# HandSomeWay/myGauHuman

Hardware: AMD Instinct MI355X
Metric: frames/sec fwd+bwd @1024^2, 200k Gaussians (higher is better)
Workload: dtype f32

## Files before the change

### mygauhuman_amd/csrc/geometry.hip

```cpp
#include "expand.h"
#include "gsr_common.h"
#include "project.h"
#include "sh_math.h"

namespace gsr {

constexpr int SH_M = 16;
constexpr int SH_ROW = SH_M * 3;
constexpr int SH_HALF = SH_ROW / 2;
constexpr int SH_LDS_ROW = 28;
constexpr int SH_CPT = SH_HALF / 4;

template <bool STAGE_SH>
__global__ __launch_bounds__(PRE_BLOCK) void preprocess_forward_kernel(const PreprocessArgs a) {
  __shared__ uint32_t wave_tot[PRE_BLOCK / WAVE];
  __shared__ __attribute__((aligned(16))) float s_sh[STAGE_SH ? PRE_BLOCK * SH_LDS_ROW : 4];
  const int i = blockIdx.x * PRE_BLOCK + threadIdx.x;
  float4 second[STAGE_SH ? SH_CPT : 1];
  if (STAGE_SH) {
    const int first = blockIdx.x * PRE_BLOCK;
    const int nrows = min(PRE_BLOCK, a.P - first);
    if (a.sh_half) {
      const uint4 *slab = reinterpret_cast<const uint4 *>(reinterpret_cast<const _Float16 *>(a.shs) + (size_t)first * SH_ROW);
#pragma unroll
// ... 54 lines not shown
        const float l1 = mid + sqrtf(fmaxf(0.1f, mid * mid - det));
        const float l2 = mid - sqrtf(fmaxf(0.1f, mid * mid - det));
        const float radf = ceilf(3.f * sqrtf(fmaxf(l1, l2)));
        const float pix = ndc2pix(pprojx, a.W), piy = ndc2pix(pprojy, a.H);
        int x0, y0, x1, y1;
        const int radi = f2i_sat(radf);
        tile_rect(pix, piy, radi, a.grid_x, a.grid_y, x0, y0, x1, y1);
        const uint32_t area = (uint32_t)(x1 - x0) * (uint32_t)(y1 - y0);
        if (area != 0) {
          float3 rgb = make_float3(0.f, 0.f, 0.f);
          if (a.colors_precomp) {
            rgb = make_float3(a.colors_precomp[3 * (size_t)i], a.colors_precomp[3 * (size_t)i + 1], a.colors_precomp[3 * (size_t)i + 2]);
          } else if (STAGE_SH) {
            want_sh = true;
          } else {
            rgb = sh_to_rgb(a.D, p, a.campos, a.shs + (size_t)i * a.M * 3, clamp_bits);
          }
          my_radius = radi;
          tiles = area;
          rec.x = pix;
          rec.y = piy;
          rec.conic_a = cv.z * det_inv;
          rec.conic_b = -cv.y * det_inv;
          rec.conic_c = cv.x * det_inv;
          rec.opacity = a.opacities[i];
          rec.depth = pv.z;
          rec.r = rgb.x;
          rec.g = rgb.y;
          rec.b = rgb.z;
          const float o = rec.opacity, t255 = 255.0f * o;
          float hx = __builtin_inff(), hy = __builtin_inff();
// ... 4 lines not shown
              const float tau2 = 2.0f * (logf(t255) + 0.02f);
              hx = sqrtf(tau2 * cv.x) * 1.0001f + 0.01f;
              hy = sqrtf(tau2 * cv.z) * 1.0001f + 0.01f;
            }
          }
          rec.hx = hx;
          rec.hy = hy;
        }
      }
    }
  }
  if (STAGE_SH) {
    float3 d0;
    const ShDir dir = sh_dir(p, a.campos, d0);
    float res[3] = {0.f, 0.f, 0.f};
    __syncthreads();
    if (want_sh) sh_accumulate<0, SH_M / 2>(a.D, dir, &s_sh[threadIdx.x * SH_LDS_ROW], res);
    __syncthreads();
    {
      const int nrows = min(PRE_BLOCK, a.P - blockIdx.x * PRE_BLOCK);
      if (a.sh_half) {
#pragma unroll
        for (int j = 0; j < SH_CPT / 2; j++) {
          const int e = (int)threadIdx.x + j * PRE_BLOCK, row = e / (SH_CPT / 2), c8 = e % (SH_CPT / 2);
          if (row < nrows) {
            const _Float16 *hv = reinterpret_cast<const _Float16 *>(&second[j]);
            float *dst = &s_sh[row * SH_LDS_ROW + 8 * c8];
#pragma unroll
            for (int e2 = 0; e2 < 8; e2++) dst[e2] = (float)hv[e2];
          }
        }
      } else {
#pragma unroll
        for (int j = 0; j < SH_CPT; j++) {
          const int e = (int)threadIdx.x + j * PRE_BLOCK, row = e / SH_CPT, c4 = e % SH_CPT;
          if (row < nrows) *reinterpret_cast<float4 *>(&s_sh[row * SH_LDS_ROW + 4 * c4]) = second[j];
        }
      }
    }
    __syncthreads();
    if (want_sh) {
      sh_accumulate<SH_M / 2, SH_M>(a.D, dir, &s_sh[threadIdx.x * SH_LDS_ROW], res);
      const float3 rgb = sh_finish(res, clamp_bits);
      rec.r = rgb.x;
      rec.g = rgb.y;
      rec.b = rgb.z;
    }
  }
  if (i < a.P) {
    a.radii[i] = my_radius;
    a.geom.tiles_touched[i] = tiles;
    a.geom.clamped[i] = (uint8_t)clamp_bits;
    float4 *dst = reinterpret_cast<float4 *>(a.geom.recs + i);
    dst[0] = make_float4(rec.x, rec.y, rec.conic_a, rec.conic_b);
    dst[1] = make_float4(rec.conic_c, rec.opacity, rec.depth, rec.r);
    dst[2] = make_float4(rec.g, rec.b, rec.hx, rec.hy);
    if (a.zero_rows) {
      float4 *row = reinterpret_cast<float4 *>(a.geom.grad_rows + (size_t)i * GROWX);
#pragma unroll
      for (int k = 0; k < GROWX / 4; k++) row[k] = make_float4(0.f, 0.f, 0.f, 0.f);
    }
// ... 137 lines not shown
```

### mygauhuman_amd/csrc/gsr_api.hip

```cpp
#include <stdarg.h>
#include <stdio.h>
#include <string.h>

#include <atomic>
#include <mutex>
#include <string>
#include <unordered_map>
#include <utility>
#include <vector>

#include "gsr_common.h"

namespace gsr {

static thread_local std::string g_error;

void set_error(const char *fmt, ...) {
  char buf[1024];
  va_list ap;
  va_start(ap, fmt);
  vsnprintf(buf, sizeof(buf), fmt, ap);
  va_end(ap);
  g_error = buf;
}
// ... 638 lines not shown
      !dL_dcov3D) {
    set_error("gsr_rasterize_backward: null required pointer");
    return GSR_EINVAL;
  }
  if (p1 && (n_extra != CE_MAX || !p1->gt_image || !p1->gt_normal || !p1->alpha_target || !p1->bound || !p1->color || !p1->alpha ||
             !p1->extra_images || !p1->stats || p1->normal_triple < 0 || p1->normal_triple > 5 || p1->axis_triple < 0 ||
             p1->axis_triple > 5 || p1->axis_triple == p1->normal_triple)) {
    set_error("gsr_rasterize_backward_phase1_loss: the fused multi-feature pass (n_extra = %d), the forward's images, the targets, "
              "the bound mask, stats and two different triple indices in 0..5 are required", CE_MAX);
    return GSR_EINVAL;
  }
  if ((shs && !dL_dsh) || (scales && (!rotations || !dL_dscale || !dL_drot))) {
    set_error("gsr_rasterize_backward: missing gradient output for SH / scale / rotation inputs");
    return GSR_EINVAL;
  }
  const int grid_x = (width + TILE - 1) / TILE, grid_y = (height + TILE - 1) / TILE;
  const size_t tiles = (size_t)grid_x * grid_y, npix = (size_t)width * height;
  GeomState geom = geom_from_chunk(geom_buffer, (size_t)P);
  BinningState bin = binning_from_chunk(binning_buffer, (size_t)R);
  ImageState img = image_from_chunk(image_buffer, npix, tiles);
  if (!radii) radii = geom.internal_radii;

  if (n_extra != 0 && (n_extra != CE_MAX || !extra_features || !dL_dout_extra || !dL_dextra)) {
    set_error("gsr_rasterize_backward_ex: extra feature channels need n_extra == %d and all three arrays", CE_MAX);
    return GSR_EINVAL;
  }
  const int grow = n_extra ? GROWX : GROW;
  const Options opt = options_for(stream);
  float *det_rows = nullptr;
  const size_t det_bytes = (size_t)(R > 0 ? R : 1) * 4 * GROW * sizeof(float);
// ... 68 lines not shown
      (void)hipFree(det_rows);
    }
    return rc;
  }
  GSR_LAUNCH_CHECK(stream, debug);

  PreprocessBwdArgs pb;
  memset(&pb, 0, sizeof(pb));
  pb.P = P;
  pb.D = D;
  pb.M = M;
  pb.means3D = means3D;
  pb.shs = shs;
  pb.scales = scales;
  pb.rotations = rotations;
  pb.cov3D = cov3D_precomp ? cov3D_precomp : geom.cov3D;
  pb.radii = radii;
  pb.clamped = geom.clamped;
  pb.scale_modifier = scale_modifier;
  pb.view = viewmatrix;
  pb.proj = projmatrix;
  pb.campos = campos;
  pb.W = width;
  pb.H = height;
  pb.tan_fovx = tan_fovx;
  pb.tan_fovy = tan_fovy;
  pb.focal_y = height / (2.0f * tan_fovy);
  pb.focal_x = width / (2.0f * tan_fovx);
  pb.grad_rows = geom.grad_rows;
  pb.grow = grow;
  pb.clear_rows = (flags & GSR_BWD_ROWS_ZEROED) ? 1 : 0;
  pb.CE = n_extra;
  pb.sh_half = sh_dtype == GSR_SH_F16 ? 1 : 0;
// ... 257 lines not shown
```

### mygauhuman_amd/csrc/gsr_common.h

```cpp
#pragma once
#include <hip/hip_runtime.h>
#include <stdint.h>
#include <stddef.h>

#include "../../include/gsr.h"

namespace gsr {

constexpr int TILE = 16;
constexpr int WAVE = 64;
constexpr int PRE_BLOCK = 256;

struct alignas(16) SplatRec {
  float x, y, conic_a, conic_b;
  float conic_c, opacity, depth, r;
  float g, b, hx, hy;
};
static_assert(sizeof(SplatRec) == 48, "SplatRec layout");

constexpr int GROW = 16;

constexpr int GROWX = 32;
constexpr int CE_MAX = 18;

struct GeomState {
  SplatRec *recs;
  float *cov3D;
  uint8_t *clamped;
  uint32_t *tiles_touched;
  uint32_t *point_offsets;
  int *internal_radii;
  uint32_t *block_incl;
  uint32_t *block_sums;
  uint32_t *block_prefix;
  uint32_t *total;
  float *grad_rows;
};
struct BinningState {
  uint64_t *keys_a;
  uint32_t *vals_a;
  uint64_t *keys_s;
  uint32_t *vals_s;
  uint32_t *hist;
// ... 20 lines not shown

inline int pre_blocks(int P) { return (P + PRE_BLOCK - 1) / PRE_BLOCK; }
constexpr int SORT_ITEMS = 16;
constexpr int SORT_BLOCK = 256;
constexpr int SORT_TILE = SORT_ITEMS * SORT_BLOCK;
inline size_t sort_blocks(size_t n) { return (n + SORT_TILE - 1) / SORT_TILE; }
inline size_t sort_hist_words(size_t n) { return 256 * (sort_blocks(n) ? sort_blocks(n) : 1) + 256; }

inline GeomState geom_from_chunk(char *chunk_, size_t P, size_t *end = nullptr) {
  GeomState g;
  uintptr_t chunk = carve_begin(chunk_);
  size_t nb = (size_t)pre_blocks((int)P);
  carve(chunk, g.recs, P);
  carve(chunk, g.cov3D, P * 6);
  carve(chunk, g.clamped, P);
  carve(chunk, g.tiles_touched, P);
  carve(chunk, g.point_offsets, P);
  carve(chunk, g.internal_radii, P);
  carve(chunk, g.block_incl, P);
  carve(chunk, g.block_sums, nb);
  carve(chunk, g.block_prefix, nb);
  carve(chunk, g.total, 4);
  carve(chunk, g.grad_rows, P * GROWX);
  if (end) *end = chunk;
  return g;
}
inline size_t geom_bytes(size_t P) {
  size_t end = 0;
  geom_from_chunk(nullptr, P, &end);
  return end + 256;
// ... 225 lines not shown
  const float *g_img[CB_IMAGES];
  int n_img;
  uint64_t col0;
  uint32_t col_mask;
  float *dL_dextra;
  float *dL_dcolor;
  int list_prio;
};
int launch_blend_colors_backward(const BlendColorsBwdArgs &a, hipStream_t stream);

struct PreprocessBwdArgs {
  int P, D, M;
  const float *means3D, *shs, *scales, *rotations, *cov3D;
  const int *radii;
  const uint8_t *clamped;
  float scale_modifier;
  const float *view, *proj, *campos;
  int W, H;
  float tan_fovx, tan_fovy, focal_x, focal_y;
  float *grad_rows;
  int grow;
  int clear_rows;
  int CE;
  float *dL_dextra;
  const SplatRec *recs;
  float *dL_dmean2D, *dL_dconic, *dL_dopacity, *dL_dcolor, *dL_dmean3D, *dL_dcov3D, *dL_dsh, *dL_dscale, *dL_drot;
  int sh_half;
};
int launch_preprocess_backward(const PreprocessBwdArgs &a, hipStream_t stream);

// ... 104 lines not shown
```

### mygauhuman_amd/csrc/preprocess_bwd.hip

```cpp
#include "gsr_common.h"
#include "sh_math.h"

namespace gsr {

__device__ __forceinline__ void cov3d_backward(const float3 sc, float mod, const float4 q, const float *d, float *dL_dscale,
                                               float *dL_drot) {
  const float r = q.x, x = q.y, y = q.z, z = q.w;
  float R[3][3];
  R[0][0] = 1.f - 2.f * (y * y + z * z);
  R[0][1] = 2.f * (x * y - r * z);
  R[0][2] = 2.f * (x * z + r * y);
  R[1][0] = 2.f * (x * y + r * z);
  R[1][1] = 1.f - 2.f * (x * x + z * z);
  R[1][2] = 2.f * (y * z - r * x);
  R[2][0] = 2.f * (x * z - r * y);
  R[2][1] = 2.f * (y * z + r * x);
  R[2][2] = 1.f - 2.f * (x * x + y * y);
  const float s[3] = {mod * sc.x, mod * sc.y, mod * sc.z};
  float M[3][3];
#pragma unroll
  for (int c = 0; c < 3; c++)
#pragma unroll
    for (int rr = 0; rr < 3; rr++) M[c][rr] = s[rr] * R[c][rr];
  const float dS[3][3] = {{d[0], 0.5f * d[1], 0.5f * d[2]}, {0.5f * d[1], d[3], 0.5f * d[4]}, {0.5f * d[2], 0.5f * d[4], d[5]}};
// ... 6 lines not shown
#pragma unroll
  for (int k = 0; k < 3; k++) dL_dscale[k] = R[0][k] * dMt[k][0] + R[1][k] * dMt[k][1] + R[2][k] * dMt[k][2];
#pragma unroll
  for (int k = 0; k < 3; k++)
#pragma unroll
    for (int rr = 0; rr < 3; rr++) dMt[k][rr] *= s[k];
  dL_drot[0] = 2 * z * (dMt[0][1] - dMt[1][0]) + 2 * y * (dMt[2][0] - dMt[0][2]) + 2 * x * (dMt[1][2] - dMt[2][1]);
  dL_drot[1] = 2 * y * (dMt[1][0] + dMt[0][1]) + 2 * z * (dMt[2][0] + dMt[0][2]) + 2 * r * (dMt[1][2] - dMt[2][1]) -
               4 * x * (dMt[2][2] + dMt[1][1]);
  dL_drot[2] = 2 * x * (dMt[1][0] + dMt[0][1]) + 2 * r * (dMt[2][0] - dMt[0][2]) + 2 * z * (dMt[1][2] + dMt[2][1]) -
               4 * y * (dMt[2][2] + dMt[0][0]);
  dL_drot[3] = 2 * r * (dMt[0][1] - dMt[1][0]) + 2 * x * (dMt[2][0] + dMt[0][2]) + 2 * y * (dMt[1][2] + dMt[2][1]) -
               4 * z * (dMt[1][1] + dMt[0][0]);
}

struct DeferredSh {
  bool live;
  float3 mean;
  float dRGB[3];
  float dm[3];
};

template <bool DEFER_SH>
__device__ __forceinline__ void preprocess_backward_one(const PreprocessBwdArgs &a, int i, const float *sh_in, float *dsh_out,
                                                        DeferredSh *out) {
  if (DEFER_SH) out->live = false;
  if (!(a.radii[i] > 0)) {
#pragma unroll
    for (int k = 0; k < 3; k++) {
      a.dL_dmean2D[3 * (size_t)i + k] = 0.f;
      a.dL_dcolor[3 * (size_t)i + k] = 0.f;
      a.dL_dmean3D[3 * (size_t)i + k] = 0.f;
      if (a.scales) a.dL_dscale[3 * (size_t)i + k] = 0.f;
    }
#pragma unroll
    for (int k = 0; k < 4; k++) {
      a.dL_dconic[4 * (size_t)i + k] = 0.f;
      if (a.scales) a.dL_drot[4 * (size_t)i + k] = 0.f;
    }
    a.dL_dopacity[i] = 0.f;
// ... 28 lines not shown
  a.dL_dmean2D[3 * (size_t)i + 1] = g0.y;
  a.dL_dmean2D[3 * (size_t)i + 2] = 0.f;
  a.dL_dconic[4 * (size_t)i + 0] = g0.z;
  a.dL_dconic[4 * (size_t)i + 1] = g0.w;
  a.dL_dconic[4 * (size_t)i + 2] = 0.f;
  a.dL_dconic[4 * (size_t)i + 3] = g1.x;
  a.dL_dopacity[i] = g1.y;
  a.dL_dcolor[3 * (size_t)i + 0] = g1.z;
  a.dL_dcolor[3 * (size_t)i + 1] = g1.w;
  a.dL_dcolor[3 * (size_t)i + 2] = g2.x;
  const float dcx = g0.z, dcy = g0.w, dcz = g1.x;

  const float *vm = a.view, *proj = a.proj;
  const float3 mean = make_float3(a.means3D[3 * (size_t)i], a.means3D[3 * (size_t)i + 1], a.means3D[3 * (size_t)i + 2]);
  float c6[6];
#pragma unroll
  for (int k = 0; k < 6; k++) c6[k] = a.cov3D[6 * (size_t)i + k];

  float3 t = make_float3(vm[0] * mean.x + vm[4] * mean.y + vm[8] * mean.z + vm[12],
                         vm[1] * mean.x + vm[5] * mean.y + vm[9] * mean.z + vm[13],
                         vm[2] * mean.x + vm[6] * mean.y + vm[10] * mean.z + vm[14]);
  const float limx = 1.3f * a.tan_fovx, limy = 1.3f * a.tan_fovy;
  const float txtz = t.x / t.z, tytz = t.y / t.z;
  t.x = fminf(limx, fmaxf(-limx, txtz)) * t.z;
  t.y = fminf(limy, fmaxf(-limy, tytz)) * t.z;
  const float gxm = (txtz < -limx || txtz > limx) ? 0.f : 1.f;
  const float gym = (tytz < -limy || tytz > limy) ? 0.f : 1.f;
  const float h_x = a.focal_x, h_y = a.focal_y;
  const float J00 = h_x / t.z, J02 = -(h_x * t.x) / (t.z * t.z), J11 = h_y / t.z, J12 = -(h_y * t.y) / (t.z * t.z);
  const float Wm[3][3] = {{vm[0], vm[4], vm[8]}, {vm[1], vm[5], vm[9]}, {vm[2], vm[6], vm[10]}};
  float T[2][3];
#pragma unroll
// ... 49 lines not shown
  const float dtz = -h_x * tz2 * dJ00 - h_y * tz2 * dJ11 + (2 * h_x * t.x) * tz3 * dJ02 + (2 * h_y * t.y) * tz3 * dJ12;
  float dm[3];
  dm[0] = vm[0] * dtx + vm[1] * dty + vm[2] * dtz;
  dm[1] = vm[4] * dtx + vm[5] * dty + vm[6] * dtz;
  dm[2] = vm[8] * dtx + vm[9] * dty + vm[10] * dtz;

  const float mhw = proj[3] * mean.x + proj[7] * mean.y + proj[11] * mean.z + proj[15];
  const float m_w = 1.0f / (mhw + 0.0000001f);
  const float mul1 = (proj[0] * mean.x + proj[4] * mean.y + proj[8] * mean.z + proj[12]) * m_w * m_w;
  const float mul2 = (proj[1] * mean.x + proj[5] * mean.y + proj[9] * mean.z + proj[13]) * m_w * m_w;
  const float g2x = g0.x, g2y = g0.y;
  dm[0] += (proj[0] * m_w - proj[3] * mul1) * g2x + (proj[1] * m_w - proj[3] * mul2) * g2y;
  dm[1] += (proj[4] * m_w - proj[7] * mul1) * g2x + (proj[5] * m_w - proj[7] * mul2) * g2y;
  dm[2] += (proj[8] * m_w - proj[11] * mul1) * g2x + (proj[9] * m_w - proj[11] * mul2) * g2y;

  if (DEFER_SH) {
    const uint32_t cb = a.clamped[i];
    out->live = true;
    out->mean = mean;
    out->dRGB[0] = (cb & 1u) ? 0.f : g1.z;
    out->dRGB[1] = (cb & 2u) ? 0.f : g1.w;
    out->dRGB[2] = (cb & 4u) ? 0.f : g2.x;
    out->dm[0] = dm[0];
    out->dm[1] = dm[1];
    out->dm[2] = dm[2];
  } else {
    if (a.shs) {
      sh_backward(a.D, mean, a.campos, sh_in, a.clamped[i], make_float3(g1.z, g1.w, g2.x), dm, dsh_out);
      for (int k = (a.D + 1) * (a.D + 1) * 3; k < a.M * 3; k++) dsh_out[k] = 0.f;
    }
    a.dL_dmean3D[3 * (size_t)i + 0] = dm[0];
    a.dL_dmean3D[3 * (size_t)i + 1] = dm[1];
    a.dL_dmean3D[3 * (size_t)i + 2] = dm[2];
  }

  if (a.scales) {
    float ds[3], dq[4];
    const float3 sc = make_float3(a.scales[3 * (size_t)i], a.scales[3 * (size_t)i + 1], a.scales[3 * (size_t)i + 2]);
    const float4 q = make_float4(a.rotations[4 * (size_t)i], a.rotations[4 * (size_t)i + 1], a.rotations[4 * (size_t)i + 2],
                                 a.rotations[4 * (size_t)i + 3]);
    cov3d_backward(sc, a.scale_modifier, q, dcov, ds, dq);
#pragma unroll
    for (int k = 0; k < 3; k++) a.dL_dscale[3 * (size_t)i + k] = ds[k];
#pragma unroll
    for (int k = 0; k < 4; k++) a.dL_drot[4 * (size_t)i + k] = dq[k];
  }
}

constexpr int BSH_M = 16, BSH_ROW = BSH_M * 3;
constexpr int BSH_HALF = BSH_ROW / 2;
constexpr int BSH_LDS_ROW = 28;
constexpr int BSH_CPT = BSH_HALF / 4;
constexpr int BWD_BLOCK = 128;

template <bool STAGE_SH>
__global__ __launch_bounds__(BWD_BLOCK) void preprocess_backward_kernel(const PreprocessBwdArgs a) {
  __shared__ __attribute__((aligned(16))) float s_sh[STAGE_SH ? BWD_BLOCK * BSH_LDS_ROW : 4];
  const int i = blockIdx.x * BWD_BLOCK + threadIdx.x;
  if (a.CE > 0) {
    const int first = blockIdx.x * BWD_BLOCK;
    const int nrows = min(BWD_BLOCK, a.P - first);
    const float *src = a.grad_rows + (size_t)first * a.grow + 9;
    float *dst = a.dL_dextra + (size_t)first * a.CE;
    for (int e = threadIdx.x; e < nrows * a.CE; e += BWD_BLOCK) {
      const int r = e / a.CE, c = e - r * a.CE;
      dst[e] = src[(size_t)r * a.grow + c];
    }
    if (a.clear_rows) {
      __syncthreads();
      float *rows = a.grad_rows + (size_t)first * a.grow;
      for (int e = threadIdx.x; e < nrows * (a.grow - 12); e += BWD_BLOCK) {
        const int r = e / (a.grow - 12), c = e - r * (a.grow - 12);
        rows[(size_t)r * a.grow + 12 + c] = 0.f;
      }
    }
  }
  if (STAGE_SH) {
    const int first = blockIdx.x * BWD_BLOCK;
    const int nrows = min(BWD_BLOCK, a.P - first);
    float4 second[BSH_CPT];
    if (a.sh_half) {
      const uint4 *slab = reinterpret_cast<const uint4 *>(reinterpret_cast<const _Float16 *>(a.shs) + (size_t)first * BSH_ROW);
#pragma unroll
      for (int j = 0; j < BSH_CPT / 2; j++) {
        const int e = (int)threadIdx.x + j * BWD_BLOCK, row = e / (BSH_CPT / 2), c8 = e % (BSH_CPT / 2);
        if (row < nrows) {
          const uint4 v = slab[row * (BSH_ROW / 8) + c8];
          second[j] = __builtin_bit_cast(float4, slab[row * (BSH_ROW / 8) + BSH_CPT / 2 + c8]);
          const _Float16 *hv = reinterpret_cast<const _Float16 *>(&v);
          float *dst = &s_sh[row * BSH_LDS_ROW + 8 * c8];
#pragma unroll
          for (int e2 = 0; e2 < 8; e2++) dst[e2] = (float)hv[e2];
        }
      }
    } else {
      const float4 *slab = reinterpret_cast<const float4 *>(a.shs + (size_t)first * BSH_ROW);
#pragma unroll
      for (int j = 0; j < BSH_CPT; j++) {
        const int e = (int)threadIdx.x + j * BWD_BLOCK, row = e / BSH_CPT, c4 = e % BSH_CPT;
        if (row < nrows) {
          *reinterpret_cast<float4 *>(&s_sh[row * BSH_LDS_ROW + 4 * c4]) = slab[row * (BSH_ROW / 4) + c4];
          second[j] = slab[row * (BSH_ROW / 4) + BSH_CPT + c4];
        }
      }
    }
    DeferredSh d;
    d.live = false;
    if (i < a.P) preprocess_backward_one<true>(a, i, nullptr, nullptr, &d);
    float3 d0 = make_float3(1.f, 0.f, 0.f);
    ShDir dir = {};
    float dd[9] = {0.f, 0.f, 0.f, 0.f, 0.f, 0.f, 0.f, 0.f, 0.f};
    if (d.live) dir = sh_dir(d.mean, a.campos, d0);
    float *mine = &s_sh[threadIdx.x * BSH_LDS_ROW];
    float4 *out = reinterpret_cast<float4 *>(a.dL_dsh + (size_t)first * BSH_ROW);
    __syncthreads();
    if (d.live) {
      sh_backward_range<0, BSH_M / 2>(a.D, dir, mine, d.dRGB, dd);
    } else if (i < a.P) {
#pragma unroll
      for (int k = 0; k < BSH_HALF; k++) mine[k] = 0.f;
    }
    __syncthreads();
#pragma unroll
    for (int j = 0; j < BSH_CPT; j++) {
      const int e = (int)threadIdx.x + j * BWD_BLOCK, row = e / BSH_CPT, c4 = e % BSH_CPT;
      if (row < nrows) {
        float4 *cell = reinterpret_cast<float4 *>(&s_sh[row * BSH_LDS_ROW + 4 * c4]);
        out[row * (BSH_ROW / 4) + c4] = *cell;
        if (!a.sh_half) *cell = second[j];
      }
    }
    if (a.sh_half) {
      __syncthreads();
#pragma unroll
      for (int j = 0; j < BSH_CPT / 2; j++) {
        const int e = (int)threadIdx.x + j * BWD_BLOCK, row = e / (BSH_CPT / 2), c8 = e % (BSH_CPT / 2);
        if (row < nrows) {
          const _Float16 *hv = reinterpret_cast<const _Float16 *>(&second[j]);
          float *dst = &s_sh[row * BSH_LDS_ROW + 8 * c8];
#pragma unroll
          for (int e2 = 0; e2 < 8; e2++) dst[e2] = (float)hv[e2];
        }
      }
    }
    __syncthreads();
    if (d.live) {
      sh_backward_range<BSH_M / 2, BSH_M>(a.D, dir, mine, d.dRGB, dd);
      sh_backward_finish(d0, d.dRGB, dd, d.dm);
      a.dL_dmean3D[3 * (size_t)i + 0] = d.dm[0];
      a.dL_dmean3D[3 * (size_t)i + 1] = d.dm[1];
      a.dL_dmean3D[3 * (size_t)i + 2] = d.dm[2];
    } else if (i < a.P) {
#pragma unroll
      for (int k = 0; k < BSH_HALF; k++) mine[k] = 0.f;
    }
    __syncthreads();
#pragma unroll
    for (int j = 0; j < BSH_CPT; j++) {
      const int e = (int)threadIdx.x + j * BWD_BLOCK, row = e / BSH_CPT, c4 = e % BSH_CPT;
      if (row < nrows) out[row * (BSH_ROW / 4) + BSH_CPT + c4] = *reinterpret_cast<const float4 *>(&s_sh[row * BSH_LDS_ROW + 4 * c4]);
    }
  } else {
    if (i < a.P)
      preprocess_backward_one<false>(a, i, a.shs ? a.shs + (size_t)i * a.M * 3 : nullptr,
                                     a.shs ? a.dL_dsh + (size_t)i * a.M * 3 : nullptr, nullptr);
  }
}

int launch_preprocess_backward(const PreprocessBwdArgs &a, hipStream_t stream) {
  if (a.P <= 0) return GSR_OK;
  const bool stage = a.shs && a.M == BSH_M && (reinterpret_cast<size_t>(a.shs) % 16 == 0) &&
                     (reinterpret_cast<size_t>(a.dL_dsh) % 16 == 0);
  if (a.sh_half && a.shs && !stage) {
    set_error("fp16 SH storage needs 16 coefficients per Gaussian and 16-byte aligned arrays");
    return GSR_EINVAL;
  }
  if (stage)
    hipLaunchKernelGGL(preprocess_backward_kernel<true>, dim3((a.P + BWD_BLOCK - 1) / BWD_BLOCK), dim3(BWD_BLOCK), 0, stream, a);
  else
    hipLaunchKernelGGL(preprocess_backward_kernel<false>, dim3((a.P + BWD_BLOCK - 1) / BWD_BLOCK), dim3(BWD_BLOCK), 0, stream, a);
  return GSR_OK;
}

}
```

### mygauhuman_amd/csrc/sh_math.h

```cpp
#pragma once
#include "gsr_common.h"

namespace gsr {

constexpr float kSH0 = 0.28209479177387814f;
constexpr float kSH1 = 0.4886025119029199f;
constexpr float kSH2[5] = {1.0925484305920792f, -1.0925484305920792f, 0.31539156525252005f, -1.0925484305920792f,
                           0.5462742152960396f};
constexpr float kSH3[7] = {-0.5900435899266435f, 2.890611442640554f, -0.4570457994644658f, 0.3731763325901154f,
                           -0.4570457994644658f, 1.445305721320277f,  -0.5900435899266435f};

__device__ __forceinline__ float3 sh_to_rgb(int deg, const float3 pos, const float *campos, const float *sh,
                                            uint32_t &clamp_bits) {
  const float dx0 = pos.x - campos[0], dy0 = pos.y - campos[1], dz0 = pos.z - campos[2];
  const float len = sqrtf(dx0 * dx0 + dy0 * dy0 + dz0 * dz0);
  const float x = dx0 / len, y = dy0 / len, z = dz0 / len;
  float out[3];
  clamp_bits = 0;
#pragma unroll
  for (int ch = 0; ch < 3; ch++) {
#define S(k) sh[(k) * 3 + ch]
    float res = kSH0 * S(0);
    if (deg > 0) {
      res = res - kSH1 * y * S(1) + kSH1 * z * S(2) - kSH1 * x * S(3);
// ... 175 lines not shown
    sh_accumulate<LO, HI, K + 1>(deg, d, part, res);
  }
}
__device__ __forceinline__ float3 sh_finish(float (&res)[3], uint32_t &clamp_bits) {
  clamp_bits = 0;
#pragma unroll
  for (int ch = 0; ch < 3; ch++) {
    res[ch] += 0.5f;
    if (res[ch] < 0) clamp_bits |= 1u << ch;
    res[ch] = fmaxf(res[ch], 0.0f);
  }
  return make_float3(res[0], res[1], res[2]);
}

template <int LO, int HI, int K = LO>
__device__ __forceinline__ void sh_backward_range(int deg, const ShDir &d, float *part, const float (&dRGB)[3], float (&dd)[9]) {
  if constexpr (K < HI) {
    float *c = part + (K - LO) * 3;
    if (deg >= sh_band_of(K)) {
      const float w = sh_weight<K>(d);
      if constexpr (K > 0) {
        const float3 g = sh_weight_grad<K>(d);
#pragma unroll
        for (int ch = 0; ch < 3; ch++) {
          const float s = c[ch];
          dd[ch] += g.x * s;
          dd[3 + ch] += g.y * s;
          dd[6 + ch] += g.z * s;
        }
      }
#pragma unroll
      for (int ch = 0; ch < 3; ch++) c[ch] = w * dRGB[ch];
    } else {
      c[0] = c[1] = c[2] = 0.f;
    }
    sh_backward_range<LO, HI, K + 1>(deg, d, part, dRGB, dd);
  }
}
__device__ __forceinline__ void sh_backward_finish(const float3 d0, const float (&dRGB)[3], const float (&dd)[9], float *dL_dmean) {
  const float dd0 = dd[0] * dRGB[0] + dd[1] * dRGB[1] + dd[2] * dRGB[2];
  const float dd1 = dd[3] * dRGB[0] + dd[4] * dRGB[1] + dd[5] * dRGB[2];
  const float dd2 = dd[6] * dRGB[0] + dd[7] * dRGB[1] + dd[8] * dRGB[2];
  const float sum2 = d0.x * d0.x + d0.y * d0.y + d0.z * d0.z;
  const float inv32 = 1.0f / sqrtf(sum2 * sum2 * sum2);
  dL_dmean[0] += ((+sum2 - d0.x * d0.x) * dd0 - d0.y * d0.x * dd1 - d0.z * d0.x * dd2) * inv32;
  dL_dmean[1] += (-d0.x * d0.y * dd0 + (sum2 - d0.y * d0.y) * dd1 - d0.z * d0.y * dd2) * inv32;
  dL_dmean[2] += (-d0.x * d0.z * dd0 - d0.y * d0.z * dd1 + (sum2 - d0.z * d0.z) * dd2) * inv32;
}

__device__ __forceinline__ void sh_basis(int deg, float x, float y, float z, float *w) {
  w[0] = kSH0;
// ... 26 lines not shown
```

### mygauhuman_amd/diff_gaussian_rasterization/_C.py

```python
import contextlib
import ctypes as C

import torch

from .. import _lib
from .._lib import ALLOC_FN, call, check, lib, ptr
from ..fastpath import DeferredStatus


def _f32c(t, name):
    if t.numel() and t.dtype != torch.float32:
        raise RuntimeError(f"{name} must be float32")
    return t.contiguous()


def _sh(t):
    if t.numel() and t.dtype == torch.float16:
        return t.contiguous(), _lib.SH_F16
    return _f32c(t, "sh"), _lib.SH_F32


class _Scratch:

    def __init__(self, device):
        self.device = device
        self.tensor = torch.empty(0, dtype=torch.uint8, device=device)
        self.error = None
        self.cb = ALLOC_FN(self._alloc)

    def _alloc(self, _user, nbytes):
        try:
            self.tensor = torch.empty(int(nbytes), dtype=torch.uint8, device=self.device)
            return self.tensor.data_ptr()
        except Exception as ex:
# ... 209 lines not shown
            raise RuntimeError(f"Phase1Loss: targets must be {H}x{W} images on {dev}")
    stats = torch.empty((8,), dtype=torch.float32, device=dev)
    if spec._partials is None or spec._partials.device != dev:
        spec._partials = torch.empty((int(lib.gsr_phase1_loss_partials()),), dtype=torch.float32, device=dev)
    st = spec.struct(_f32c(color, "color"), _f32c(alpha, "alpha"), _f32c(out_extra, "out_extra"), stats)
    call("gsr_phase1_loss_forward", dev, W, H, C.byref(st), spec._partials.data_ptr())
    return stats[0], stats


def rasterize_gaussians_backward(background, means3D, radii, colors, scales, rotations, scale_modifier, cov3D_precomp,
                                 viewmatrix, projmatrix, tan_fovx, tan_fovy, dL_dout_color, dL_dout_depth,
                                 dL_dout_alpha, sh, degree, campos, geomBuffer, R, binningBuffer, imageBuffer, alphas,
                                 debug, out=None, extra=None, dL_dout_extra=None, phase1=None):
    dev = means3D.device
    P, H, W = means3D.size(0), alphas.size(-2), alphas.size(-1)
    M = sh.size(1) if sh.numel() != 0 else 0
    opts = dict(dtype=torch.float32, device=dev)
    new = torch.zeros if P == 0 else torch.empty
    has_sr = scales.numel() != 0
    out = out or {}

    def _get(name, shape, alloc):
        t = out.get(name)
        if t is None:
            return alloc(shape, **opts)
        if tuple(t.shape) != tuple(shape) or t.dtype != torch.float32 or not t.is_contiguous() or t.device != dev:
            raise RuntimeError(f"out['{name}'] must be a contiguous float32 tensor of shape {tuple(shape)} on {dev}")
        return t

    dL_dmeans3D = _get("means3D", (P, 3), new)
# ... 40 lines not shown
            ptr(dL_dout_alpha), dL_dmeans2D.data_ptr(), dL_dconic.data_ptr(), dL_dopacity.data_ptr(),
            dL_dcolors.data_ptr(), dL_dmeans3D.data_ptr(), dL_dcov3D.data_ptr(),
            dL_dsh.data_ptr() if M else None, None if dL_dscales is None else dL_dscales.data_ptr(),
            None if dL_drotations is None else dL_drotations.data_ptr(), int(bool(debug)),
            ptr(extra), 0 if extra is None else _lib.N_EXTRA, None if extra is None else extra_ptrs,
            None if dL_dextra is None else dL_dextra.data_ptr(), sh_dtype, *loss)
    if extra is not None:
        return dL_dmeans2D, dL_dcolors, dL_dopacity, dL_dmeans3D, dL_dcov3D, dL_dsh, dL_dscales, dL_drotations, dL_dextra
    return dL_dmeans2D, dL_dcolors, dL_dopacity, dL_dmeans3D, dL_dcov3D, dL_dsh, dL_dscales, dL_drotations


def rasterize_gaussians_backward_colors(P, R, image_height, image_width, geomBuffer, binningBuffer, imageBuffer, dL_dout_color=None,
                                        dL_dout_extra=None, debug=False, out=None):
    dev = geomBuffer.device
    P, H, W = int(P), int(image_height), int(image_width)
    opts = dict(dtype=torch.float32, device=dev)
    out = out or {}

    def _get(name, shape):
        t = out.get(name)
        if t is None:
            return (torch.zeros if P == 0 else torch.empty)(shape, **opts)
        if tuple(t.shape) != tuple(shape) or t.dtype != torch.float32 or not t.is_contiguous() or t.device != dev:
            raise RuntimeError(f"out['{name}'] must be a contiguous float32 tensor of shape {tuple(shape)} on {dev}")
        return t

    def _image(g, planes, name):
        if g is None:
            return None
        if tuple(g.shape) != (planes, H, W) or g.device != dev:
# ... 18 lines not shown


def mark_visible(means3D, viewmatrix, projmatrix):
    if not means3D.is_cuda:
        raise RuntimeError("mark_visible: tensors must live on a HIP device (no CPU path)")
    P = means3D.size(0)
    present = torch.zeros((P,), dtype=torch.bool, device=means3D.device)
    if P != 0:
        means3D, viewmatrix, projmatrix = _f32c(means3D, "means3D"), _f32c(viewmatrix, "viewmatrix"), _f32c(projmatrix, "projmatrix")
        call("gsr_mark_visible", means3D.device, P, ptr(means3D), ptr(viewmatrix), ptr(projmatrix), present.data_ptr())
    return present


def query_state(what, P, R, W, H, geomBuffer, binningBuffer, imageBuffer):
    dev = geomBuffer.device
    tiles = ((W + 15) // 16) * ((H + 15) // 16)
    shapes = dict(DEPTHS=((P,), torch.float32), MEANS2D=((P, 2), torch.float32), CONIC_OPACITY=((P, 4), torch.float32),
                  RGB=((P, 3), torch.float32), COV3D=((P, 6), torch.float32), TILES_TOUCHED=((P,), torch.int32),
                  POINT_OFFSETS=((P,), torch.int32), CLAMPED=((P, 3), torch.uint8), POINT_LIST=((R,), torch.int32),
                  KEYS_SORTED=((R,), torch.int64), RANGES=((tiles, 2), torch.int32), FINAL_T=((H, W), torch.float32),
                  N_CONTRIB=((H, W), torch.int32), ORDER=((4 * tiles + 66,), torch.int32))
    shape, dt = shapes[what]
    out = torch.zeros(shape, dtype=dt, device=dev)
    if out.numel():
        call("gsr_query_state", dev, _lib.Q[what], P, R, W, H, geomBuffer.data_ptr(),
             binningBuffer.data_ptr() if binningBuffer.numel() else None, imageBuffer.data_ptr(), out.data_ptr())
    return out
```

### mygauhuman_amd/fastpath.py

```python
import dataclasses

import torch

from ._lib import SH_F16, SH_F32, call, lib

ROWS_ZEROED = 2


@dataclasses.dataclass(eq=False)
class Deferred:
    index: int
    tag: object
    words: torch.Tensor
    event: torch.cuda.Event


class DeferredStatus:

    def __init__(self, n_words, decide):
        self.n_words, self.decide = int(n_words), decide
        self.issued = 0
        self.pending = []
        self._words, self._events = [], []

# ... 61 lines not shown
        R = _C.rasterize_gaussians(bg, params["means3D"], e, params["opacities"], params["scales"], params["rotations"], 1.0,
                                   e, cam["viewmatrix"], cam["projmatrix"], cam["tanfovx"], cam["tanfovy"], cam["H"], cam["W"],
                                   params["shs"], sh_degree, cam["campos"], False, False)[0]
        P, M = params["means3D"].shape[0], params["shs"].shape[1]
        return RasterSession(P, cam["W"], cam["H"], M, params["means3D"].device, int(R * slack) + 4096, with_backward)

    def regrown(self, capacity):
        if capacity <= self.capacity:
            return self
        n = RasterSession.__new__(RasterSession)
        n.__dict__.update(self.__dict__)
        n.capacity = int(capacity)
        n.bin = torch.empty(lib.gsr_binning_bytes(n.capacity, n.W, n.H), dtype=torch.uint8, device=n.device)
        return n

    def _stream(self):
        return torch.cuda.current_stream(self.device).cuda_stream

    def forward(self, params, cam, bg, sh_degree, scale_modifier=1.0):
        p = params
        sh_dtype = SH_F16 if p["shs"].dtype == torch.float16 else SH_F32
        call(
            "gsr_rasterize_forward_async_ex", None,
            self.geom.data_ptr(), self.bin.data_ptr(), self.capacity, self.img.data_ptr(), self.P, int(sh_degree), self.M,
            bg.data_ptr(), self.W, self.H, p["means3D"].data_ptr(), p["shs"].data_ptr(), None, p["opacities"].data_ptr(),
            p["scales"].data_ptr(), float(scale_modifier), p["rotations"].data_ptr(), None, cam["viewmatrix"].data_ptr(),
            cam["projmatrix"].data_ptr(), cam["campos"].data_ptr(), float(cam["tanfovx"]), float(cam["tanfovy"]), 0,
            self.color.data_ptr(), self.depth.data_ptr(), self.alpha.data_ptr(), self.radii.data_ptr(), 0,
            self.status.data_ptr(), None, 0, None, sh_dtype, stream=self._stream())
        return self.color, self.depth, self.alpha, self.radii

    def alpha_mask_loss_backward(self, gt, mask, lambda_alpha=0.1):
        call("gsr_alpha_mask_loss_backward", None, self.W, self.H, self.color.data_ptr(), self.alpha.data_ptr(), gt.data_ptr(),
             mask.data_ptr(), float(lambda_alpha), self.dL_dcolor.data_ptr(), self.dL_dalpha.data_ptr(), stream=self._stream())
        return self.dL_dcolor, self.dL_dalpha

    def backward(self, params, cam, bg, sh_degree, dL_dcolor, dL_ddepth, dL_dalpha, out, scale_modifier=1.0):
        p = params
        sh_dtype = SH_F16 if p["shs"].dtype == torch.float16 else SH_F32
        call(
            "gsr_rasterize_backward_ex", None,
            self.P, int(sh_degree), self.M, self.capacity, bg.data_ptr(), self.W, self.H, p["means3D"].data_ptr(),
            p["shs"].data_ptr(), None, self.alpha.data_ptr(), p["scales"].data_ptr(), float(scale_modifier),
            p["rotations"].data_ptr(), None, cam["viewmatrix"].data_ptr(), cam["projmatrix"].data_ptr(),
            cam["campos"].data_ptr(), float(cam["tanfovx"]), float(cam["tanfovy"]), self.radii.data_ptr(),
            self.geom.data_ptr(), self.bin.data_ptr(), self.img.data_ptr(), dL_dcolor.data_ptr(), dL_ddepth.data_ptr(),
            dL_dalpha.data_ptr(), self.dL_dmean2D.data_ptr(), self.dL_dconic.data_ptr(), out["opacity"].data_ptr(),
            self.dL_dcolors.data_ptr(), out["means3D"].data_ptr(), self.dL_dcov3D.data_ptr(), out["sh"].data_ptr(),
            out["scales"].data_ptr(), out["rotations"].data_ptr(), ROWS_ZEROED, None, 0, None, None, sh_dtype,
            stream=self._stream())

    def backward_alpha_mask_loss(self, params, cam, bg, sh_degree, gt, mask, lambda_alpha, out, scale_modifier=1.0):
        p = params
        sh_dtype = SH_F16 if p["shs"].dtype == torch.float16 else SH_F32
        call(
            "gsr_rasterize_backward_alpha_mask_loss", None,
            self.P, int(sh_degree), self.M, self.capacity, bg.data_ptr(), self.W, self.H, p["means3D"].data_ptr(),
            p["shs"].data_ptr(), None, self.alpha.data_ptr(), p["scales"].data_ptr(), float(scale_modifier),
            p["rotations"].data_ptr(), None, cam["viewmatrix"].data_ptr(), cam["projmatrix"].data_ptr(),
            cam["campos"].data_ptr(), float(cam["tanfovx"]), float(cam["tanfovy"]), self.radii.data_ptr(),
            self.geom.data_ptr(), self.bin.data_ptr(), self.img.data_ptr(), self.color.data_ptr(), gt.data_ptr(), mask.data_ptr(),
            float(lambda_alpha), self.dL_dmean2D.data_ptr(), self.dL_dconic.data_ptr(), out["opacity"].data_ptr(),
            self.dL_dcolors.data_ptr(), out["means3D"].data_ptr(), self.dL_dcov3D.data_ptr(), out["sh"].data_ptr(),
            out["scales"].data_ptr(), out["rotations"].data_ptr(), ROWS_ZEROED, sh_dtype, stream=self._stream())

    def _status_word(self, k):
        if not self.status.is_cuda:
            torch.cuda.synchronize(self.device)
        return int(self.status[k].item())
# ... 7 lines not shown
```

Measured before the change: 2850.

## Cache SH direction-gradient partials in forward; skip SH reload in backward preprocess

The forward preprocess now computes the 9-float SH direction-gradient term per Gaussian and stores it in a new geometry-buffer slot. The backward preprocess reads that cached term instead of reloading and re-staging all SH coefficients, so it only writes dL_dsh. The backward also rebuilds cov3D from scale and rotation instead of reading the stored covariance. This trades a smaller backward read volume for extra forward work, a per-Gaussian 36-byte write, and a larger geometry buffer, with new Python-side size checks.

Result: no change. 2827 (-0.8%).

```diff
diff --git a/mygauhuman_amd/csrc/geometry.hip b/mygauhuman_amd/csrc/geometry.hip
--- a/mygauhuman_amd/csrc/geometry.hip
+++ b/mygauhuman_amd/csrc/geometry.hip
@@ -92,7 +92,14 @@
           } else if (STAGE_SH) {
             want_sh = true;
           } else {
-            rgb = sh_to_rgb(a.D, p, a.campos, a.shs + (size_t)i * a.M * 3, clamp_bits);
+            const float *sh = a.shs + (size_t)i * a.M * 3;
+            rgb = sh_to_rgb(a.D, p, a.campos, sh, clamp_bits);
+            float3 d0;
+            const ShDir dir = sh_dir(p, a.campos, d0);
+            float dd[9] = {0.f, 0.f, 0.f, 0.f, 0.f, 0.f, 0.f, 0.f, 0.f};
+            sh_ddir_range<0, SH_M>(a.D, dir, sh, dd);
+#pragma unroll
+            for (int k = 0; k < 9; k++) a.geom.sh_ddir[9 * (size_t)i + k] = dd[k];
           }
           my_radius = radi;
           tiles = area;
@@ -127,8 +134,12 @@
     float3 d0;
     const ShDir dir = sh_dir(p, a.campos, d0);
     float res[3] = {0.f, 0.f, 0.f};
-    __syncthreads();
-    if (want_sh) sh_accumulate<0, SH_M / 2>(a.D, dir, &s_sh[threadIdx.x * SH_LDS_ROW], res);
+    float dd[9] = {0.f, 0.f, 0.f, 0.f, 0.f, 0.f, 0.f, 0.f, 0.f};
+    __syncthreads();
+    if (want_sh) {
+      sh_accumulate<0, SH_M / 2>(a.D, dir, &s_sh[threadIdx.x * SH_LDS_ROW], res);
+      sh_ddir_range<0, SH_M / 2>(a.D, dir, &s_sh[threadIdx.x * SH_LDS_ROW], dd);
+    }
     __syncthreads();
     {
       const int nrows = min(PRE_BLOCK, a.P - blockIdx.x * PRE_BLOCK);
@@ -154,10 +165,25 @@
     __syncthreads();
     if (want_sh) {
       sh_accumulate<SH_M / 2, SH_M>(a.D, dir, &s_sh[threadIdx.x * SH_LDS_ROW], res);
+      sh_ddir_range<SH_M / 2, SH_M>(a.D, dir, &s_sh[threadIdx.x * SH_LDS_ROW], dd);
       const float3 rgb = sh_finish(res, clamp_bits);
       rec.r = rgb.x;
       rec.g = rgb.y;
       rec.b = rgb.z;
+    }
+    __syncthreads();
+#pragma unroll
+    for (int k = 0; k < 9; k++) s_sh[threadIdx.x * SH_LDS_ROW + k] = dd[k];
+    __syncthreads();
+    {
+      const int first = blockIdx.x * PRE_BLOCK;
+      const int nwords = 9 * min(PRE_BLOCK, a.P - first);
+      float *dst = a.geom.sh_ddir + 9 * (size_t)first;
+#pragma unroll
+      for (int j = 0; j < 9; j++) {
+        const int e = (int)threadIdx.x + j * PRE_BLOCK;
+        if (e < nwords) dst[e] = s_sh[(e / 9) * SH_LDS_ROW + e % 9];
+      }
     }
   }
   if (i < a.P) {
diff --git a/mygauhuman_amd/csrc/gsr_api.hip b/mygauhuman_amd/csrc/gsr_api.hip
--- a/mygauhuman_amd/csrc/gsr_api.hip
+++ b/mygauhuman_amd/csrc/gsr_api.hip
@@ -676,6 +676,14 @@
     set_error("gsr_rasterize_backward: missing gradient output for SH / scale / rotation inputs");
     return GSR_EINVAL;
   }
+  if (shs && colors_precomp) {
+    set_error("gsr_rasterize_backward: provide SHs or precomputed colours, not both");
+    return GSR_EINVAL;
+  }
+  if (!cov3D_precomp && !scales) {
+    set_error("gsr_rasterize_backward: provide scales+rotations or a precomputed 3D covariance");
+    return GSR_EINVAL;
+  }
   const int grid_x = (width + TILE - 1) / TILE, grid_y = (height + TILE - 1) / TILE;
   const size_t tiles = (size_t)grid_x * grid_y, npix = (size_t)width * height;
   GeomState geom = geom_from_chunk(geom_buffer, (size_t)P);
@@ -774,9 +782,10 @@
   pb.shs = shs;
   pb.scales = scales;
   pb.rotations = rotations;
-  pb.cov3D = cov3D_precomp ? cov3D_precomp : geom.cov3D;
+  pb.cov3D = cov3D_precomp;
   pb.radii = radii;
   pb.clamped = geom.clamped;
+  pb.sh_ddir = geom.sh_ddir;
   pb.scale_modifier = scale_modifier;
   pb.view = viewmatrix;
   pb.proj = projmatrix;
diff --git a/mygauhuman_amd/csrc/gsr_common.h b/mygauhuman_amd/csrc/gsr_common.h
--- a/mygauhuman_amd/csrc/gsr_common.h
+++ b/mygauhuman_amd/csrc/gsr_common.h
@@ -27,6 +27,7 @@
   SplatRec *recs;
   float *cov3D;
   uint8_t *clamped;
+  float *sh_ddir;
   uint32_t *tiles_touched;
   uint32_t *point_offsets;
   int *internal_radii;
@@ -77,6 +78,7 @@
   carve(chunk, g.recs, P);
   carve(chunk, g.cov3D, P * 6);
   carve(chunk, g.clamped, P);
+  carve(chunk, g.sh_ddir, P * 9);
   carve(chunk, g.tiles_touched, P);
   carve(chunk, g.point_offsets, P);
   carve(chunk, g.internal_radii, P);
@@ -332,6 +334,7 @@
   const float *means3D, *shs, *scales, *rotations, *cov3D;
   const int *radii;
   const uint8_t *clamped;
+  const float *sh_ddir;
   float scale_modifier;
   const float *view, *proj, *campos;
   int W, H;
diff --git a/mygauhuman_amd/csrc/preprocess_bwd.hip b/mygauhuman_amd/csrc/preprocess_bwd.hip
--- a/mygauhuman_amd/csrc/preprocess_bwd.hip
+++ b/mygauhuman_amd/csrc/preprocess_bwd.hip
@@ -1,4 +1,5 @@
 #include "gsr_common.h"
+#include "project.h"
 #include "sh_math.h"
 
 namespace gsr {
@@ -44,16 +45,28 @@
                4 * z * (dMt[1][1] + dMt[0][0]);
 }
 
+constexpr int BSH_M = 16, BSH_ROW = BSH_M * 3;
+constexpr int BSH_HALF = BSH_ROW / 2;
+constexpr int BSH_LDS_ROW = 28;
+constexpr int BSH_CPT = BSH_HALF / 4;
+constexpr int BWD_BLOCK = 128;
+
 struct DeferredSh {
   bool live;
-  float3 mean;
+  ShDir dir;
   float dRGB[3];
-  float dm[3];
 };
 
+__device__ __forceinline__ void sh_mean_from_cache(const PreprocessBwdArgs &a, int i, const float3 d0, const float (&dRGB)[3],
+                                                   float *dm) {
+  float dd[9];
+#pragma unroll
+  for (int k = 0; k < 9; k++) dd[k] = a.sh_ddir[9 * (size_t)i + k];
+  sh_backward_finish(d0, dRGB, dd, dm);
+}
+
 template <bool DEFER_SH>
-__device__ __forceinline__ void preprocess_backward_one(const PreprocessBwdArgs &a, int i, const float *sh_in, float *dsh_out,
-                                                        DeferredSh *out) {
+__device__ __forceinline__ void preprocess_backward_one(const PreprocessBwdArgs &a, int i, float *dsh_out, DeferredSh *out) {
   if (DEFER_SH) out->live = false;
   if (!(a.radii[i] > 0)) {
 #pragma unroll
@@ -112,8 +125,19 @@
   const float *vm = a.view, *proj = a.proj;
   const float3 mean = make_float3(a.means3D[3 * (size_t)i], a.means3D[3 * (size_t)i + 1], a.means3D[3 * (size_t)i + 2]);
   float c6[6];
-#pragma unroll
-  for (int k = 0; k < 6; k++) c6[k] = a.cov3D[6 * (size_t)i + k];
+  float3 sc = make_float3(0.f, 0.f, 0.f);
+  float4 q = make_float4(0.f, 0.f, 0.f, 0.f);
+  if (a.scales) {
+    sc = make_float3(a.scales[3 * (size_t)i], a.scales[3 * (size_t)i + 1], a.scales[3 * (size_t)i + 2]);
+    q = make_float4(a.rotations[4 * (size_t)i], a.rotations[4 * (size_t)i + 1], a.rotations[4 * (size_t)i + 2],
+                    a.rotations[4 * (size_t)i + 3]);
+  }
+  if (a.cov3D) {
+#pragma unroll
+    for (int k = 0; k < 6; k++) c6[k] = a.cov3D[6 * (size_t)i + k];
+  } else {
+    cov3d_from_scale_rot(sc, a.scale_modifier, q, c6);
+  }
 
   float3 t = make_float3(vm[0] * mean.x + vm[4] * mean.y + vm[8] * mean.z + vm[12],
                          vm[1] * mean.x + vm[5] * mean.y + vm[9] * mean.z + vm[13],
@@ -193,31 +217,32 @@
   dm[1] += (proj[4] * m_w - proj[7] * mul1) * g2x + (proj[5] * m_w - proj[7] * mul2) * g2y;
   dm[2] += (proj[8] * m_w - proj[11] * mul1) * g2x + (proj[9] * m_w - proj[11] * mul2) * g2y;
 
-  if (DEFER_SH) {
+  if (a.shs) {
     const uint32_t cb = a.clamped[i];
-    out->live = true;
-    out->mean = mean;
-    out->dRGB[0] = (cb & 1u) ? 0.f : g1.z;
-    out->dRGB[1] = (cb & 2u) ? 0.f : g1.w;
-    out->dRGB[2] = (cb & 4u) ? 0.f : g2.x;
-    out->dm[0] = dm[0];
-    out->dm[1] = dm[1];
-    out->dm[2] = dm[2];
-  } else {
-    if (a.shs) {
-      sh_backward(a.D, mean, a.campos, sh_in, a.clamped[i], make_float3(g1.z, g1.w, g2.x), dm, dsh_out);
-      for (int k = (a.D + 1) * (a.D + 1) * 3; k < a.M * 3; k++) dsh_out[k] = 0.f;
-    }
-    a.dL_dmean3D[3 * (size_t)i + 0] = dm[0];
-    a.dL_dmean3D[3 * (size_t)i + 1] = dm[1];
-    a.dL_dmean3D[3 * (size_t)i + 2] = dm[2];
-  }
+    const float dRGB[3] = {(cb & 1u) ? 0.f : g1.z, (cb & 2u) ? 0.f : g1.w, (cb & 4u) ? 0.f : g2.x};
+    float3 d0;
+    const ShDir dir = sh_dir(mean, a.campos, d0);
+    sh_mean_from_cache(a, i, d0, dRGB, dm);
+    if (DEFER_SH) {
+      out->live = true;
+      out->dir = dir;
+#pragma unroll
+      for (int c = 0; c < 3; c++) out->dRGB[c] = dRGB[c];
+    } else {
+      float w[BSH_M];
+      sh_basis(a.D, dir.x, dir.y, dir.z, w);
+      const int active = (a.D + 1) * (a.D + 1);
+      for (int k = 0; k < a.M; k++)
+#pragma unroll
+        for (int c = 0; c < 3; c++) dsh_out[3 * k + c] = k < active ? w[k] * dRGB[c] : 0.f;
+    }
+  }
+  a.dL_dmean3D[3 * (size_t)i + 0] = dm[0];
+  a.dL_dmean3D[3 * (size_t)i + 1] = dm[1];
+  a.dL_dmean3D[3 * (size_t)i + 2] = dm[2];
 
   if (a.scales) {
     float ds[3], dq[4];
-    const float3 sc = make_float3(a.scales[3 * (size_t)i], a.scales[3 * (size_t)i + 1], a.scales[3 * (size_t)i + 2]);
-    const float4 q = make_float4(a.rotations[4 * (size_t)i], a.rotations[4 * (size_t)i + 1], a.rotations[4 * (size_t)i + 2],
-                                 a.rotations[4 * (size_t)i + 3]);
     cov3d_backward(sc, a.scale_modifier, q, dcov, ds, dq);
 #pragma unroll
     for (int k = 0; k < 3; k++) a.dL_dscale[3 * (size_t)i + k] = ds[k];
@@ -225,12 +250,6 @@
     for (int k = 0; k < 4; k++) a.dL_drot[4 * (size_t)i + k] = dq[k];
   }
 }
-
-constexpr int BSH_M = 16, BSH_ROW = BSH_M * 3;
-constexpr int BSH_HALF = BSH_ROW / 2;
-constexpr int BSH_LDS_ROW = 28;
-constexpr int BSH_CPT = BSH_HALF / 4;
-constexpr int BWD_BLOCK = 128;
 
 template <bool STAGE_SH>
 __global__ __launch_bounds__(BWD_BLOCK) void preprocess_backward_kernel(const PreprocessBwdArgs a) {
@@ -257,78 +276,28 @@
   if (STAGE_SH) {
     const int first = blockIdx.x * BWD_BLOCK;
     const int nrows = min(BWD_BLOCK, a.P - first);
-    float4 second[BSH_CPT];
-    if (a.sh_half) {
-      const uint4 *slab = reinterpret_cast<const uint4 *>(reinterpret_cast<const _Float16 *>(a.shs) + (size_t)first * BSH_ROW);
-#pragma unroll
-      for (int j = 0; j < BSH_CPT / 2; j++) {
-        const int e = (int)threadIdx.x + j * BWD_BLOCK, row = e / (BSH_CPT / 2), c8 = e % (BSH_CPT / 2);
-        if (row < nrows) {
-          const uint4 v = slab[row * (BSH_ROW / 8) + c8];
-          second[j] = __builtin_bit_cast(float4, slab[row * (BSH_ROW / 8) + BSH_CPT / 2 + c8]);
-          const _Float16 *hv = reinterpret_cast<const _Float16 *>(&v);
-          float *dst = &s_sh[row * BSH_LDS_ROW + 8 * c8];
-#pragma unroll
-          for (int e2 = 0; e2 < 8; e2++) dst[e2] = (float)hv[e2];
-        }
-      }
-    } else {
-      const float4 *slab = reinterpret_cast<const float4 *>(a.shs + (size_t)first * BSH_ROW);
-#pragma unroll
-      for (int j = 0; j < BSH_CPT; j++) {
-        const int e = (int)threadIdx.x + j * BWD_BLOCK, row = e / BSH_CPT, c4 = e % BSH_CPT;
-        if (row < nrows) {
-          *reinterpret_cast<float4 *>(&s_sh[row * BSH_LDS_ROW + 4 * c4]) = slab[row * (BSH_ROW / 4) + c4];
-          second[j] = slab[row * (BSH_ROW / 4) + BSH_CPT + c4];
-        }
-      }
-    }
     DeferredSh d;
     d.live = false;
-    if (i < a.P) preprocess_backward_one<true>(a, i, nullptr, nullptr, &d);
-    float3 d0 = make_float3(1.f, 0.f, 0.f);
-    ShDir dir = {};
-    float dd[9] = {0.f, 0.f, 0.f, 0.f, 0.f, 0.f, 0.f, 0.f, 0.f};
-    if (d.live) dir = sh_dir(d.mean, a.campos, d0);
+    d.dir = {};
+    d.dRGB[0] = d.dRGB[1] = d.dRGB[2] = 0.f;
+    if (i < a.P) preprocess_backward_one<true>(a, i, nullptr, &d);
     float *mine = &s_sh[threadIdx.x * BSH_LDS_ROW];
     float4 *out = reinterpret_cast<float4 *>(a.dL_dsh + (size_t)first * BSH_ROW);
+    if (d.live) {
+      sh_grad_range<0, BSH_M / 2>(a.D, d.dir, mine, d.dRGB);
+    } else if (i < a.P) {
+#pragma unroll
+      for (int k = 0; k < BSH_HALF; k++) mine[k] = 0.f;
+    }
+    __syncthreads();
+#pragma unroll
+    for (int j = 0; j < BSH_CPT; j++) {
+      const int e = (int)threadIdx.x + j * BWD_BLOCK, row = e / BSH_CPT, c4 = e % BSH_CPT;
+      if (row < nrows) out[row * (BSH_ROW / 4) + c4] = *reinterpret_cast<const float4 *>(&s_sh[row * BSH_LDS_ROW + 4 * c4]);
+    }
     __syncthreads();
     if (d.live) {
-      sh_backward_range<0, BSH_M / 2>(a.D, dir, mine, d.dRGB, dd);
-    } else if (i < a.P) {
-#pragma unroll
-      for (int k = 0; k < BSH_HALF; k++) mine[k] = 0.f;
-    }
-    __syncthreads();
-#pragma unroll
-    for (int j = 0; j < BSH_CPT; j++) {
-      const int e = (int)threadIdx.x + j * BWD_BLOCK, row = e / BSH_CPT, c4 = e % BSH_CPT;
-      if (row < nrows) {
-        float4 *cell = reinterpret_cast<float4 *>(&s_sh[row * BSH_LDS_ROW + 4 * c4]);
-        out[row * (BSH_ROW / 4) + c4] = *cell;
-        if (!a.sh_half) *cell = second[j];
-      }
-    }
-    if (a.sh_half) {
-      __syncthreads();
-#pragma unroll
-      for (int j = 0; j < BSH_CPT / 2; j++) {
-        const int e = (int)threadIdx.x + j * BWD_BLOCK, row = e / (BSH_CPT / 2), c8 = e % (BSH_CPT / 2);
-        if (row < nrows) {
-          const _Float16 *hv = reinterpret_cast<const _Float16 *>(&second[j]);
-          float *dst = &s_sh[row * BSH_LDS_ROW + 8 * c8];
-#pragma unroll
-          for (int e2 = 0; e2 < 8; e2++) dst[e2] = (float)hv[e2];
-        }
-      }
-    }
-    __syncthreads();
-    if (d.live) {
-      sh_backward_range<BSH_M / 2, BSH_M>(a.D, dir, mine, d.dRGB, dd);
-      sh_backward_finish(d0, d.dRGB, dd, d.dm);
-      a.dL_dmean3D[3 * (size_t)i + 0] = d.dm[0];
-      a.dL_dmean3D[3 * (size_t)i + 1] = d.dm[1];
-      a.dL_dmean3D[3 * (size_t)i + 2] = d.dm[2];
+      sh_grad_range<BSH_M / 2, BSH_M>(a.D, d.dir, mine, d.dRGB);
     } else if (i < a.P) {
 #pragma unroll
       for (int k = 0; k < BSH_HALF; k++) mine[k] = 0.f;
@@ -340,17 +309,14 @@
       if (row < nrows) out[row * (BSH_ROW / 4) + BSH_CPT + c4] = *reinterpret_cast<const float4 *>(&s_sh[row * BSH_LDS_ROW + 4 * c4]);
     }
   } else {
-    if (i < a.P)
-      preprocess_backward_one<false>(a, i, a.shs ? a.shs + (size_t)i * a.M * 3 : nullptr,
-                                     a.shs ? a.dL_dsh + (size_t)i * a.M * 3 : nullptr, nullptr);
+    if (i < a.P) preprocess_backward_one<false>(a, i, a.shs ? a.dL_dsh + (size_t)i * a.M * 3 : nullptr, nullptr);
   }
 }
 
 int launch_preprocess_backward(const PreprocessBwdArgs &a, hipStream_t stream) {
   if (a.P <= 0) return GSR_OK;
-  const bool stage = a.shs && a.M == BSH_M && (reinterpret_cast<size_t>(a.shs) % 16 == 0) &&
-                     (reinterpret_cast<size_t>(a.dL_dsh) % 16 == 0);
-  if (a.sh_half && a.shs && !stage) {
+  const bool stage = a.shs && a.M == BSH_M && (reinterpret_cast<size_t>(a.dL_dsh) % 16 == 0);
+  if (a.sh_half && a.shs && (a.M != BSH_M || reinterpret_cast<size_t>(a.shs) % 16 != 0 || !stage)) {
     set_error("fp16 SH storage needs 16 coefficients per Gaussian and 16-byte aligned arrays");
     return GSR_EINVAL;
   }
diff --git a/mygauhuman_amd/csrc/sh_math.h b/mygauhuman_amd/csrc/sh_math.h
--- a/mygauhuman_amd/csrc/sh_math.h
+++ b/mygauhuman_amd/csrc/sh_math.h
@@ -213,27 +213,35 @@
 }
 
 template <int LO, int HI, int K = LO>
-__device__ __forceinline__ void sh_backward_range(int deg, const ShDir &d, float *part, const float (&dRGB)[3], float (&dd)[9]) {
+__device__ __forceinline__ void sh_ddir_range(int deg, const ShDir &d, const float *part, float (&dd)[9]) {
+  if constexpr (K < HI) {
+    if constexpr (K > 0) {
+      if (deg >= sh_band_of(K)) {
+        const float3 g = sh_weight_grad<K>(d);
+#pragma unroll
+        for (int ch = 0; ch < 3; ch++) {
+          const float s = part[(K - LO) * 3 + ch];
+          dd[ch] += g.x * s;
+          dd[3 + ch] += g.y * s;
+          dd[6 + ch] += g.z * s;
+        }
+      }
+    }
+    sh_ddir_range<LO, HI, K + 1>(deg, d, part, dd);
+  }
+}
+template <int LO, int HI, int K = LO>
+__device__ __forceinline__ void sh_grad_range(int deg, const ShDir &d, float *part, const float (&dRGB)[3]) {
   if constexpr (K < HI) {
     float *c = part + (K - LO) * 3;
     if (deg >= sh_band_of(K)) {
       const float w = sh_weight<K>(d);
-      if constexpr (K > 0) {
-        const float3 g = sh_weight_grad<K>(d);
-#pragma unroll
-        for (int ch = 0; ch < 3; ch++) {
-          const float s = c[ch];
-          dd[ch] += g.x * s;
-          dd[3 + ch] += g.y * s;
-          dd[6 + ch] += g.z * s;
-        }
-      }
 #pragma unroll
       for (int ch = 0; ch < 3; ch++) c[ch] = w * dRGB[ch];
     } else {
       c[0] = c[1] = c[2] = 0.f;
     }
-    sh_backward_range<LO, HI, K + 1>(deg, d, part, dRGB, dd);
+    sh_grad_range<LO, HI, K + 1>(deg, d, part, dRGB);
   }
 }
 __device__ __forceinline__ void sh_backward_finish(const float3 d0, const float (&dRGB)[3], const float (&dd)[9], float *dL_dmean) {
diff --git a/mygauhuman_amd/diff_gaussian_rasterization/_C.py b/mygauhuman_amd/diff_gaussian_rasterization/_C.py
--- a/mygauhuman_amd/diff_gaussian_rasterization/_C.py
+++ b/mygauhuman_amd/diff_gaussian_rasterization/_C.py
@@ -18,6 +18,13 @@
     if t.numel() and t.dtype == torch.float16:
         return t.contiguous(), _lib.SH_F16
     return _f32c(t, "sh"), _lib.SH_F32
+
+
+def _check_geom(geomBuffer, P):
+    need = int(lib.gsr_geometry_bytes(int(P))) if P else 0
+    if geomBuffer.numel() < need:
+        raise RuntimeError(f"geometry buffer of {geomBuffer.numel()} bytes, but {P} Gaussians need {need} (gsr_geometry_bytes): it was "
+                           "not written by this library's forward for this P")
 
 
 class _Scratch:
@@ -257,6 +264,7 @@
                                  debug, out=None, extra=None, dL_dout_extra=None, phase1=None):
     dev = means3D.device
     P, H, W = means3D.size(0), alphas.size(-2), alphas.size(-1)
+    _check_geom(geomBuffer, P)
     M = sh.size(1) if sh.numel() != 0 else 0
     opts = dict(dtype=torch.float32, device=dev)
     new = torch.zeros if P == 0 else torch.empty
@@ -327,6 +335,7 @@
                                         dL_dout_extra=None, debug=False, out=None):
     dev = geomBuffer.device
     P, H, W = int(P), int(image_height), int(image_width)
+    _check_geom(geomBuffer, P)
     opts = dict(dtype=torch.float32, device=dev)
     out = out or {}
 
@@ -375,6 +384,7 @@
 
 def query_state(what, P, R, W, H, geomBuffer, binningBuffer, imageBuffer):
     dev = geomBuffer.device
+    _check_geom(geomBuffer, P)
     tiles = ((W + 15) // 16) * ((H + 15) // 16)
     shapes = dict(DEPTHS=((P,), torch.float32), MEANS2D=((P, 2), torch.float32), CONIC_OPACITY=((P, 4), torch.float32),
                   RGB=((P, 3), torch.float32), COV3D=((P, 6), torch.float32), TILES_TOUCHED=((P,), torch.int32),
diff --git a/mygauhuman_amd/fastpath.py b/mygauhuman_amd/fastpath.py
--- a/mygauhuman_amd/fastpath.py
+++ b/mygauhuman_amd/fastpath.py
@@ -99,12 +99,18 @@
         n.bin = torch.empty(lib.gsr_binning_bytes(n.capacity, n.W, n.H), dtype=torch.uint8, device=n.device)
         return n
 
+    def _check_geom(self):
+        need = int(lib.gsr_geometry_bytes(self.P))
+        if self.geom.numel() < need:
+            raise RuntimeError(f"RasterSession: geometry buffer of {self.geom.numel()} bytes, but {self.P} Gaussians need {need}")
+
     def _stream(self):
         return torch.cuda.current_stream(self.device).cuda_stream
 
     def forward(self, params, cam, bg, sh_degree, scale_modifier=1.0):
         p = params
         sh_dtype = SH_F16 if p["shs"].dtype == torch.float16 else SH_F32
+        self._check_geom()
         call(
             "gsr_rasterize_forward_async_ex", None,
             self.geom.data_ptr(), self.bin.data_ptr(), self.capacity, self.img.data_ptr(), self.P, int(sh_degree), self.M,
@@ -123,6 +129,7 @@
     def backward(self, params, cam, bg, sh_degree, dL_dcolor, dL_ddepth, dL_dalpha, out, scale_modifier=1.0):
         p = params
         sh_dtype = SH_F16 if p["shs"].dtype == torch.float16 else SH_F32
+        self._check_geom()
         call(
             "gsr_rasterize_backward_ex", None,
             self.P, int(sh_degree), self.M, self.capacity, bg.data_ptr(), self.W, self.H, p["means3D"].data_ptr(),
@@ -138,6 +145,7 @@
     def backward_alpha_mask_loss(self, params, cam, bg, sh_degree, gt, mask, lambda_alpha, out, scale_modifier=1.0):
         p = params
         sh_dtype = SH_F16 if p["shs"].dtype == torch.float16 else SH_F32
+        self._check_geom()
         call(
             "gsr_rasterize_backward_alpha_mask_loss", None,
             self.P, int(sh_degree), self.M, self.capacity, bg.data_ptr(), self.W, self.H, p["means3D"].data_ptr(),
```
